# bbc/zipkin

Hardware: AMD Instinct MI355X
Metric: spans/sec into DependencyLinks (1/2/4/8 GPU) + % of HBM roofline (higher is better)
Workload: dtype u64

## Files before the change

### zipkin_amd/csrc/zk_api.cpp

```cpp
#include <hip/hip_runtime.h>
#include <string.h>

#include <new>
#include <string>
#include <utility>
#include <vector>

#include "zk_cluster.h"
#include "zk_comm.h"

#include "zk_internal.h"
#include "zk_launch.h"
#include "zk_lh_internal.h"
#include "zk_rl_internal.h"
#include "zk_rt_internal.h"

using namespace zk;

struct EventPair {
    hipEvent_t a = nullptr, b = nullptr;
};

struct zk_ctx {
    int device = 0;
// ... 47 lines not shown
    uint8_t* carry = nullptr;
    uint64_t carry_cap = 0;
    CarryState* cs = nullptr;
    bool maybe_carry = false;
    bool any_verify = false;
    std::string err;
    zk_rt* rt = nullptr;
    uint32_t rt_mode = ZK_RT_WITH_DEPS;
    zk_rl* rl = nullptr;
    zk_lh* lh = nullptr;
    std::vector<EventPair> ev_free, ev_join, ev_reduce, ev_spill, ev_fin, ev_cluster, ev_lh;
    zk_timing tm{};
};

namespace {

zk_status fail(zk_ctx* c, zk_status s, const std::string& msg) {
    if (c) c->err = msg;
    return s;
}

zk_status hip_fail(zk_ctx* c, hipError_t e, const char* where) {
    if (e == hipErrorLaunchOutOfResources && *launch_refusal())
        return fail(c, ZK_ERR_CAPACITY, std::string(where) + ": " + launch_refusal());
    return fail(c, ZK_ERR_HIP, std::string(where) + ": " + hipGetErrorString(e));
}

#define ZK_HIP(ctx, call)                                   \
    do {                                                    \
        hipError_t _e = (call);                             \
        if (_e != hipSuccess) return hip_fail(ctx, _e, #call); \
    } while (0)

#define ZK_ST(call)                        \
    do {                                   \
        const zk_status _s = (call);       \
        if (_s != ZK_OK) return _s;        \
    } while (0)

#define ZK_TRY try {
#define ZK_CATCH(ctx)                                                                      \
    }                                                                                      \
    catch (const std::bad_alloc&) {                                                        \
        return fail(ctx, ZK_ERR_CAPACITY, "host allocation failed");                       \
    }                                                                                      \
    catch (...) {                                                                          \
        return fail(ctx, ZK_ERR_INVALID_ARG, "unexpected host exception");                 \
    }

uint64_t table_bytes(uint32_t S) { return (uint64_t)S * S * kLimbs * 8 + kTableTailBytes; }

EventPair take_pair(zk_ctx* c) {
    EventPair p;
    if (!c->ev_free.empty()) {
        p = c->ev_free.back();
        c->ev_free.pop_back();
    } else {
        hipEventCreate(&p.a);
        hipEventCreate(&p.b);
    }
    return p;
}

uint64_t tiles_for(uint64_t n) { return (n + join_tile_records() - 1) / join_tile_records(); }

zk_status ensure_links(zk_ctx* c, uint32_t grid, uint64_t stride, uint64_t n) {
    const uint64_t slots = (uint64_t)grid * stride;
    const uint64_t sorted_slots = n + 64 < slots ? n + 64 : slots;
    const uint64_t sorted_bytes = sorted_slots * (reduce_compact(grid, stride) ? sizeof(uint32_t) : sizeof(uint64_t));
    const bool set_ok = slots <= c->link_slots && grid <= c->link_lists;
    const bool scratch_ok = !c->nb || (sorted_bytes <= c->sorted_bytes && grid <= c->col_off_lists);
    if (set_ok && scratch_ok) return ZK_OK;
    if (!set_ok) {
        hipFree(c->links);
        hipFree(c->link_count);
        hipFree(c->hist);
        c->links = nullptr;
        c->link_count = nullptr;
        c->hist = nullptr;
        c->link_slots = 0;
        c->link_lists = 0;
        ZK_HIP(c, hipMalloc(&c->links, slots * sizeof(uint64_t)));
        ZK_HIP(c, hipMalloc(&c->link_count, (uint64_t)grid * sizeof(uint32_t)));
        if (c->nb) ZK_HIP(c, hipMalloc(&c->hist, (uint64_t)grid * c->nb * sizeof(uint32_t)));
        c->link_slots = slots;
        c->link_lists = grid;
    }
    if (!scratch_ok) {
        const uint64_t sb = sorted_bytes > c->sorted_bytes ? sorted_bytes : c->sorted_bytes;
        const uint32_t gl = grid > c->col_off_lists ? grid : c->col_off_lists;
        hipFree(c->col_off);
        hipFree(c->sorted);
        c->col_off = nullptr;
        c->sorted = nullptr;
        c->sorted_bytes = 0;
        c->col_off_lists = 0;
        ZK_HIP(c, hipMalloc(&c->col_off, (uint64_t)gl * c->nb * sizeof(uint32_t)));
        ZK_HIP(c, hipMalloc(&c->sorted, sb));
        c->sorted_bytes = sb;
        c->col_off_lists = gl;
        if (!c->bucket_base) ZK_HIP(c, hipMalloc(&c->bucket_base, (c->nb + 1) * sizeof(uint64_t)));
    }
    return ZK_OK;
}

bool aligned(const void* p, uintptr_t a) { return ((uintptr_t)p & (a - 1)) == 0; }

zk_status ensure_spill(zk_ctx* c, uint64_t n) {
    const uint64_t need = tiles_for(n) + 1;
    if (need > c->spill_cap) {
        if (c->spill_list) ZK_HIP(c, hipFree(c->spill_list));
        uint64_t cap = need < (1ull << 16) ? (1ull << 16) : need;
        ZK_HIP(c, hipMalloc(&c->spill_list, cap * sizeof(uint64_t)));
        c->spill_cap = cap;
    }
    if (!c->spill_scratch) {
        c->spill_stride = spill_scratch_bytes_per_wg(c->max_trace);
        ZK_HIP(c, hipMalloc(&c->spill_scratch, c->spill_stride * c->spill_wgs));
    }
    return ZK_OK;
}

constexpr int kAbortShift = 48;
constexpr uint64_t kAbortUnit = 1ull << kAbortShift;

zk_status stats_sum(zk_ctx* c, uint64_t out[ST_N], uint64_t* aborted_ranks = nullptr) {
    const size_t bytes = (size_t)kStatShards * ST_N * 8;
    if (!c->h_stats) ZK_HIP(c, hipHostMalloc((void**)&c->h_stats, bytes, hipHostMallocDefault));
    if (!c->ev_stats) ZK_HIP(c, hipEventCreateWithFlags(&c->ev_stats, hipEventDisableTiming));
    const uint64_t cells = (uint64_t)c->S * c->S;
    if (c->merged)
        ZK_HIP(c, hipMemcpyAsync(c->h_stats, c->table + cells * kLimbs, kTableTailBytes, hipMemcpyDeviceToHost,
                                 c->stream));
    else
        ZK_HIP(c, hipMemcpyAsync(c->h_stats, c->stats, bytes, hipMemcpyDeviceToHost, c->stream));
    ZK_HIP(c, hipEventRecord(c->ev_stats, c->stream));
    hipError_t q;
    while ((q = hipEventQuery(c->ev_stats)) == hipErrorNotReady) {
    }
    if (q != hipSuccess) return fail(c, ZK_ERR_HIP, std::string("stats copy: ") + hipGetErrorString(q));
    const unsigned long long* h = c->h_stats;
    for (int s = 0; s < ST_N; ++s) out[s] = 0;
    for (int sh = 0; sh < (c->merged ? 1 : kStatShards); ++sh)
        for (int s = 0; s < ST_N; ++s) out[s] += h[(size_t)sh * ST_N + s];
    if (aborted_ranks) *aborted_ranks = out[ST_RECORDS] >> kAbortShift;
    out[ST_RECORDS] &= kAbortUnit - 1;
    return ZK_OK;
}

bool cols_ok(const zk_span_cols* c) {
    return c && c->trace_id && c->span_id && c->parent_id && c->first_ts && c->last_ts && c->service_id && c->flags;
}

uint64_t carved_bytes(uint64_t n) { return 5 * ((n * 8 + 255) & ~255ull) + 2 * ((n * 4 + 255) & ~255ull); }
SpanColsMut carve_cols(uint8_t* p, uint64_t n) {
    auto take = [&](uint64_t bytes) {
        uint8_t* q = p;
        p += (bytes + 255) & ~255ull;
        return q;
    };
    SpanColsMut m;
    m.trace_id = (uint64_t*)take(n * 8);
    m.span_id = (uint64_t*)take(n * 8);
    m.parent_id = (uint64_t*)take(n * 8);
    m.first_ts = (int64_t*)take(n * 8);
    m.last_ts = (int64_t*)take(n * 8);
    m.service_id = (uint32_t*)take(n * 4);
    m.flags = (uint32_t*)take(n * 4);
    return m;
}

zk_status ensure_cluster(zk_ctx* c, uint64_t n, const ClusterPlan& plan) {
    const uint64_t tb = cluster_scratch_bytes(plan);
    if (n > c->cl_cap) {
        hipFree(c->cl_cols);
        c->cl_cols = nullptr;
        c->cl_cap = 0;
        if (hipMalloc(&c->cl_cols, 2 * carved_bytes(n)) != hipSuccess) {
            (void)hipGetLastError();
            return fail(c, ZK_ERR_CAPACITY, "no device memory for the clustering pass (96 B per record)");
// ... 914 lines not shown
```

### zipkin_amd/csrc/zk_internal.h

```cpp
#pragma once
#include <hip/hip_runtime.h>
#include <stdint.h>

#include <string>

#include "../../include/zkagg.h"

#include <rocprofiler-sdk-roctx/roctx.h>
namespace zk {
struct RoctxRange {
    explicit RoctxRange(const char* name) { roctxRangePushA(name); }
    ~RoctxRange() { roctxRangePop(); }
    RoctxRange(const RoctxRange&) = delete;
    RoctxRange& operator=(const RoctxRange&) = delete;
};
}

namespace zk {

constexpr int kLimbs = 16;
constexpr int kLimbM0 = 0;
constexpr int kLimbS1 = 1;
constexpr int kLimbS2 = 3;
constexpr int kLimbS3 = 6;
// ... 24 lines not shown
    ST_RT_DUR_RANGE,
    ST_SPILL_OVERFLOW,
    ST_NOT_CLUSTERED,
    ST_N = 16
};
constexpr int kStatShards = 256;
constexpr uint64_t kTableTailBytes = ST_N * 8;
constexpr uint64_t kStatTailWords = ST_N;
static_assert(ST_NOT_CLUSTERED < ST_N, "stat slots");

struct SpanColsDev {
    const uint64_t* trace_id;
    const uint64_t* span_id;
    const uint64_t* parent_id;
    const int64_t* first_ts;
    const int64_t* last_ts;
    const uint32_t* service_id;
    const uint32_t* flags;
    uint64_t n;
};

struct JoinArgs {
    SpanColsDev c;
    uint64_t* table;
    unsigned long long* stats;
    uint32_t S;
    unsigned int* spill_count;
    uint64_t* spill_list;
    uint64_t spill_cap;
    uint8_t* spill_scratch;
    uint64_t spill_scratch_stride;
    uint32_t max_trace;
    uint64_t* links;
    uint32_t* link_count;
    uint64_t link_stride;
    uint64_t per_wg;
    uint32_t grid;
    uint32_t* hist;
    uint32_t nb;
    uint32_t cb_shift;
    uint32_t join;
    uint32_t skip;
    uint64_t* rt_pay;
    uint32_t* rt_svc;
    uint32_t* rt_count;
    unsigned long long* rt_dropped;
    uint64_t rt_spill_cap;
    uint64_t rt_seed;
    uint32_t rt_p;
    const uint32_t* sub;
    uint32_t nsub;
    uint32_t* big_list;
    unsigned int* big_count;
    const unsigned long long* n_dev;
    uint32_t append;
    const uint32_t* skip_dev;
    uint64_t* lk_key;
    uint64_t* lk_tid;
    uint32_t* lk_spill_count;
    uint64_t lk_spill_cap;
    uint32_t* lk_name;
    uint32_t* lh_hist;
    uint32_t lh_bins;
    uint32_t lh_m;
};

hipError_t launch_join(const JoinArgs& a, hipStream_t s, uint32_t blocks = 0);
hipError_t launch_group_join(const JoinArgs& a, hipStream_t s);
void group_join_geometry(uint64_t n, uint32_t cus, uint32_t* grid, uint64_t* per_wg, uint64_t* link_stride);
uint32_t group_join_capacity();
uint64_t join_tile_records();
void join_geometry(uint64_t n, uint32_t cus, uint32_t* grid, uint64_t* per_wg, uint64_t* link_stride);
hipError_t launch_link_reduce(const uint64_t* links, const uint32_t* counts, uint64_t stride, uint64_t tiles,
                              uint64_t* table, hipStream_t s);
#ifndef ZK_COMPACT_SLOT_LIMIT
#define ZK_COMPACT_SLOT_LIMIT 0x7FFFFFFFull
#endif
constexpr uint64_t kCompactSlotLimit = ZK_COMPACT_SLOT_LIMIT;
static_assert(kCompactSlotLimit <= 0x7FFFFFFFull, "an escape holds the slot in 31 bits, all ones is the pad");
constexpr uint32_t kCompactDurBits = 21;
constexpr uint32_t kCompactDurMask = (1u << kCompactDurBits) - 1;
constexpr uint32_t kCompactEscape = 0x80000000u;
constexpr uint32_t kCompactPad = 0xFFFFFFFFu;
bool reduce_compact(uint32_t lists, uint64_t stride);
struct ReduceArgs {
    const uint64_t* links;
    const uint32_t* counts;
    uint64_t stride;
    uint32_t lists;
    const uint32_t* hist;
    uint32_t nb, cb_shift;
    uint32_t* col_off;
    uint64_t* bucket_base;
    void* sorted;
    uint64_t* table;
    uint64_t cells;
    uint32_t compact;
};
hipError_t launch_partitioned_reduce(const ReduceArgs& r, hipStream_t s);
void bucket_geometry(uint32_t S, uint32_t* nb, uint32_t* cb_shift);
uint64_t reduce_scatter_dyn_lds(uint32_t S);
uint32_t scatter_lists_per_wg(uint32_t lists);
hipError_t launch_spill(const JoinArgs& a, uint32_t spill_wgs, hipStream_t s);
uint64_t spill_scratch_bytes_per_wg(uint32_t max_trace);
hipError_t launch_finalize(const uint64_t* table, uint32_t S, const zk_link_table* out,
                           hipStream_t s);
uint64_t exchange_bytes(uint32_t S);
hipError_t launch_table_pack(const uint64_t* table, uint32_t S, uint64_t* xchg, hipStream_t s);
hipError_t launch_table_unpack(const uint64_t* xchg, uint32_t S, uint64_t* table, hipStream_t s);
hipError_t launch_tracegen(const zk_tracegen_params* p, const zk_span_cols* out, uint64_t cap,
                           uint64_t* n_records, uint64_t* n_traces, hipStream_t s);

}
```

### zipkin_amd/csrc/zk_join.hip

```cpp
#include "zk_internal.h"
#include "zk_launch.h"
#include "zk_sketch_internal.h"

#ifndef ZK_HASH_FACTOR
#define ZK_HASH_FACTOR 8
#endif
#ifndef ZK_K1_WGS_PER_CU
#define ZK_K1_WGS_PER_CU 4
#endif
namespace zk {
namespace {

constexpr int kSpillWG = 256;

#ifdef ZK_STAMPS
__device__ unsigned long long g_zk_stamps[16];
__device__ __forceinline__ unsigned long long zk_memtime() {
    unsigned long long t;
    __builtin_amdgcn_sched_barrier(0);
    asm volatile("s_memtime %0\n\ts_waitcnt lgkmcnt(0)" : "=s"(t)::"memory");
    __builtin_amdgcn_sched_barrier(0);
    return t;
}
#define ZK_STAMP_DECL                                 \
// ... 215 lines not shown
__device__ __forceinline__ uint32_t lanes_below(uint64_t m) {
    return __builtin_amdgcn_mbcnt_hi((uint32_t)(m >> 32), __builtin_amdgcn_mbcnt_lo((uint32_t)m, 0u));
}

struct Window {
    uint64_t tid[2], sid[2], pid[2], first[2], last[2];
    uint32_t svc[2], flags[2];
    uint64_t prev;
};

__device__ __forceinline__ void window_ballots(const Window& w, uint64_t ws, int wn, uint64_t* ev, uint64_t* od) {
    const int t = threadIdx.x, lane = t & 63;
    uint64_t prev = lane_shr1(w.tid[1]);
    if (lane == 0) prev = (ws + 2 * t > 0) ? w.prev : ~w.tid[0];
    const bool b0 = (2 * t < wn) && w.tid[0] != prev;
    const bool b1 = (2 * t + 1 < wn) && w.tid[1] != w.tid[0];
    *ev = __ballot(b0);
    *od = __ballot(b1);
}

__device__ __forceinline__ void load_tid(const JoinArgs& a, uint64_t n, uint64_t ws, Window& w) {
    const uint64_t i = ws + 2 * threadIdx.x;
    ld2_u64(a.c.trace_id, i, n, w.tid);
    w.prev = a.c.trace_id[ZK_HOTIDX((i > 0 && i - 1 < n) ? i - 1 : 0)];
}
__device__ __forceinline__ void load_early(const JoinArgs& a, uint64_t n, uint64_t ws, Window& w) {
    const uint64_t i = ws + 2 * threadIdx.x;
    ld2_u64(a.c.span_id, i, n, w.sid);
#ifndef ZK_K1_DIAG_NOFIRST
    ld2_u64((const uint64_t*)a.c.first_ts, i, n, w.first);
#endif
    ld2_u64((const uint64_t*)a.c.last_ts, i, n, w.last);
#ifdef ZK_K1_DIAG_NOFIRST
    w.first[0] = w.last[0] - 5;
    w.first[1] = w.last[1] - 5;
#endif
    ld2_u32(a.c.service_id, i, n, w.svc);
}
template <bool JOIN>
__device__ __forceinline__ void load_late(const JoinArgs& a, uint64_t n, uint64_t ws, Window& w) {
    const uint64_t i = ws + 2 * threadIdx.x;
    if constexpr (JOIN) {
        ld2_u64(a.c.parent_id, i, n, w.pid);
    } else {
        w.pid[0] = w.pid[1] = 0ull;
    }
    ld2_u32(a.c.flags, i, n, w.flags);
}

constexpr int kModeJoin = 1;
constexpr int kModeEmit = 2;
constexpr int kModeLinks = 4;
template <int TILE, int WG, int MODE>
__global__ __launch_bounds__(WG, ZK_K1_WGS_PER_CU * WG / 256) void k_span_join_stream(JoinArgs a) {
    constexpr int H = ZK_HASH_FACTOR * TILE;
    constexpr int NWORD = TILE / 64;
    static_assert(TILE == 2 * WG && TILE <= 512, "two records per thread; the segment field of the slot word is 9 bits");
    __shared__ __align__(16) uint64_t s_sid[TILE];
    __shared__ __align__(16) long long s_first[TILE];
    __shared__ __align__(16) long long s_last[TILE];
    __shared__ __align__(16) uint64_t s_pid[TILE];
    __shared__ __align__(16) uint32_t s_svck[TILE];
    __shared__ __align__(16) uint32_t s_name[(MODE & kModeLinks) ? TILE / 2 : 1];
    __shared__ __align__(16) uint32_t s_ht[H];
    __shared__ __align__(16) uint64_t s_mask[NWORD];
    __shared__ uint32_t s_stat[ST_N];
    __shared__ uint64_t s_cursor;
    __shared__ uint32_t s_hist[kMaxBuckets];

    const int tid = threadIdx.x, lane = tid & 63, wave = tid >> 6;
    const uint64_t n = a.n_dev ? (uint64_t)*a.n_dev : a.c.n;
    uint64_t per = a.per_wg;
    if (a.n_dev) {
        const uint64_t q = ((n + a.grid - 1) / a.grid + TILE - 1) / TILE * TILE;
        if (q < per) per = q ? q : TILE;
    }
    const uint64_t R0 = (uint64_t)blockIdx.x * per;
    if (R0 >= n) {
        if (a.append) return;
        if (tid == 0) {
            a.link_count[blockIdx.x] = 0u;
            if (a.rt_count) a.rt_count[blockIdx.x] = 0u;
        }
        for (uint32_t x = tid; x < a.nb; x += WG) a.hist[(uint64_t)x * a.grid + blockIdx.x] = 0u;
        return;
    }
    const uint64_t R1 = (R0 + per < n) ? R0 + per : n;
    uint64_t* __restrict__ out = a.links + (uint64_t)blockIdx.x * a.link_stride;
    const uint64_t trash = a.link_stride - 1;
    uint64_t* __restrict__ it_pay = a.rt_pay + (uint64_t)blockIdx.x * a.link_stride;
    uint32_t* __restrict__ it_svc = a.rt_svc + (uint64_t)blockIdx.x * a.link_stride;
    uint64_t nrec = 0;
    StatPack st;
    int fold_in = kFoldWindows;
    if (tid < ST_N) s_stat[tid] = 0u;
    if (tid == 0) s_cursor = a.append ? (uint64_t)a.link_count[blockIdx.x] : 0ull;
    for (uint32_t x = tid; x < a.nb; x += WG) s_hist[x] = a.append ? a.hist[(uint64_t)x * a.grid + blockIdx.x] : 0u;
    constexpr uint32_t kNoSlot = 0xFFFFFFFFu;
    uint32_t r_clear[2] = {kNoSlot, kNoSlot};

    Window cur, nxt;
    constexpr bool JOIN = (MODE & kModeJoin) != 0, EMIT = (MODE & kModeEmit) != 0, LINKS = (MODE & kModeLinks) != 0;
    static_assert(!LINKS || (JOIN && !EMIT), "link items ride on the join's links");
#pragma unroll
    for (int x = tid; x < H / 4; x += WG) reinterpret_cast<uint4*>(s_ht)[x] = make_uint4(0u, 0u, 0u, 0u);
    uint64_t m_ev, m_od;
    ZK_STAMP_DECL
    uint64_t ws = R0;
    const uint32_t skip0 = a.skip_dev ? *a.skip_dev : a.skip;
    uint64_t seek = R0 + (blockIdx.x == 0 ? skip0 : 0u);
    bool seek_start = false;
    load_tid(a, n, ws, cur);
    load_early(a, n, ws, cur);
    window_ballots(cur, ws, (int)((n - ws) < (uint64_t)TILE ? (n - ws) : (uint64_t)TILE), &m_ev, &m_od);
    if (lane == 0) *reinterpret_cast<ulonglong2*>(&s_mask[2 * wave]) = make_ulonglong2(m_ev, m_od);
    for (;;) {
        load_late<JOIN>(a, n, ws, cur);
        const int wn = (int)((n - ws) < (uint64_t)TILE ? (n - ws) : (uint64_t)TILE);
        ZK_PHASE_SYNC(0);
        const int lo_j = (int)(seek - ws);
        const int r1_j = (R1 - ws < (uint64_t)wn) ? (int)(R1 - ws) : wn;
        int start = -1, stop = -1, last_b = -1, prev_b = -1;
        {
            constexpr int NW = WG / 64;
            uint64_t ev = 0ull, od = 0ull;
            if (lane < NW) {
                const ulonglong2 x = *reinterpret_cast<const ulonglong2*>(&s_mask[2 * lane]);
                ev = x.x;
                od = x.y;
            }
            const int base = 128 * lane;
            const bool fast = seek_start && lo_j < wn && R1 - ws >= (uint64_t)wn;
            if (fast) {
                start = lo_j;
            } else {
                const int fs = lane < NW ? first_ge(ev, od, lo_j - base) : -1;
                const int ft = lane < NW ? first_ge(ev, od, r1_j - base) : -1;
                const uint64_t bs = __ballot(fs >= 0), bt = __ballot(ft >= 0);
                if (bs) {
                    const int w = __ffsll((unsigned long long)bs) - 1;
                    start = 128 * w + __builtin_amdgcn_readlane(fs, w);
                }
                if (bt) {
                    const int w = __ffsll((unsigned long long)bt) - 1;
                    stop = 128 * w + __builtin_amdgcn_readlane(ft, w);
                }
            }
            const int lb = last_of(ev, od);
            const uint64_t bl = __ballot(lb >= 0);
            if (bl) {
                const int w = 63 - (int)__clzll((long long)bl);
                last_b = 128 * w + __builtin_amdgcn_readlane(lb, w);
            }
            const uint64_t bp = bl & ((1ull << wave) - 1ull);
            if (bp) {
                const int w = 63 - (int)__clzll((long long)bp);
                prev_b = 128 * w + __builtin_amdgcn_readlane(lb, w);
            }
        }
        const bool at_end = ws + (uint64_t)wn >= n;
        int m;
        bool done = false;
        uint64_t next_seek = 0;
        bool next_seek_start = false;
        if (start < 0 || (stop >= 0 && stop <= start)) {
            done = (start >= 0) || at_end || ws + (uint64_t)TILE >= R1;
            next_seek = ws + (uint64_t)TILE;
            start = m = 0;
        } else if (stop >= 0) {
            m = stop;
            done = true;
        } else if (at_end) {
            m = wn;
            done = true;
        } else if (last_b > start) {
            m = last_b;
            next_seek = ws + (uint64_t)last_b;
            next_seek_start = true;
        } else if (start > 1) {
            m = start;
// ... 214 lines not shown
        {
            const uint64_t wtot = (uint64_t)(__popcll(l1) + __popcll(l2)) | ((uint64_t)(__popcll(i1) + __popcll(i2)) << 32);
            uint64_t old = 0;
            if (lane == 0 && wtot) old = atomicAdd((unsigned long long*)&s_cursor, (unsigned long long)wtot);
            old = ((uint64_t)(uint32_t)__shfl((int)(uint32_t)(old >> 32), 0) << 32) | (uint32_t)__shfl((int)(uint32_t)old, 0);
            lbase = (uint32_t)old + lanes_below(l1) + lanes_below(l2);
            ibase = (uint32_t)(old >> 32) + lanes_below(i1) + lanes_below(i2);
        }
        if (!done) {
            const uint64_t nws = next_ws;
            window_ballots(nxt, nws, (int)((n - nws) < (uint64_t)TILE ? (n - nws) : (uint64_t)TILE), &n_ev, &n_od);
            if (lane == 0) *reinterpret_cast<ulonglong2*>(&s_mask[2 * wave]) = make_ulonglong2(n_ev, n_od);
        }
        if constexpr (JOIN) {
            uint32_t pos = lbase;
#if defined(ZK_K1_DIAG_TRASHONLY)
            out[trash] = r_link[0];
            out[trash] = r_link[1];
#elif !defined(ZK_K1_DIAG_NOSTORE)
#pragma unroll
            for (int e = 0; e < 2; ++e) {
                const bool v = (lm >> e) & 1u;
                const uint64_t at = v ? (uint64_t)pos : trash;
                out[at] = r_link[e];
                if constexpr (LINKS) {
                    a.lk_key[(uint64_t)blockIdx.x * a.link_stride + at] = r_lkey[e];
                    a.lk_tid[(uint64_t)blockIdx.x * a.link_stride + at] = cur.tid[e];
                    a.lk_name[(uint64_t)blockIdx.x * a.link_stride + at] = r_lname[e];
                }
                pos += v ? 1u : 0u;
            }
#else
            if (pos == 0xFFFFFFFFu) out[0] = r_link[0];
#endif
        }
        if constexpr (EMIT) {
            uint32_t pos = ibase;
#pragma unroll
            for (int e = 0; e < 2; ++e) {
                const bool v = r_item[e] != ~0ull;
                const uint64_t at = v ? (uint64_t)pos : trash;
                it_pay[at] = r_item[e];
                it_svc[at] = r_isvc[e];
                pos += v ? 1u : 0u;
            }
        }
#pragma unroll
        for (int e = 0; e < 2; ++e) r_clear[e] = (r_leader[e] == 2 * tid + e) ? r_slot[e] : kNoSlot;
        ZK_STAMP(6);
        if (--fold_in == 0) {
            fold_stats(st, s_stat);
            fold_in = kFoldWindows;
        }
        if (done) break;
        ws = next_ws;
        seek = next_seek;
        seek_start = next_seek_start;
        m_ev = n_ev;
        m_od = n_od;
        cur.tid[0] = nxt.tid[0];
        cur.tid[1] = nxt.tid[1];
        cur.prev = nxt.prev;
        ZK_STAMP(7);
    }
    ZK_STAMP_FLUSH();
    __syncthreads();
#ifdef ZK_K1_DIAG
    if (tid == 0) s_cursor = 0ull;
    for (uint32_t x = tid; x < a.nb; x += WG) s_hist[x] = 0u;
    __syncthreads();
#endif
    const uint32_t nout = (uint32_t)s_cursor;
    const uint32_t nitem = (uint32_t)(s_cursor >> 32);
    if (tid == 0) {
        a.link_count[blockIdx.x] = nout;
        if constexpr (EMIT) a.rt_count[blockIdx.x] = nitem;
        atomicAdd(&a.stats[(uint64_t)(blockIdx.x % kStatShards) * ST_N + ST_RECORDS], (unsigned long long)nrec);
    }
    fold_stats(st, s_stat);
    publish_stats(s_stat, a.stats);
    if constexpr (EMIT) {
        if (tid == 0 && s_stat[ST_RT_DUR_RANGE]) atomicAdd(&a.rt_dropped[1], (unsigned long long)s_stat[ST_RT_DUR_RANGE]);
    }
    if constexpr (JOIN) {
        for (uint32_t x = tid; x < a.nb; x += WG) a.hist[(uint64_t)x * a.grid + blockIdx.x] = s_hist[x];
    } else {
        for (uint32_t x = tid; x < a.nb; x += WG) a.hist[(uint64_t)x * a.grid + blockIdx.x] = 0u;
    }
}

struct SpillScratch {
    uint64_t* sid;
    long long* first;
    long long* last;
    uint64_t* cntA;
    uint64_t* cntB;
    uint64_t* pid;
    uint32_t* svck;
    uint32_t* name;
    uint32_t* ht;
};

__host__ __device__ inline uint64_t pow2ceil(uint64_t x) {
    uint64_t p = 1;
    while (p < x) p <<= 1;
    return p;
}

__host__ __device__ inline uint64_t spill_ht_slots(uint32_t max_trace) { return pow2ceil(2ull * max_trace); }

__host__ __device__ inline SpillScratch spill_carve(uint8_t* base, uint32_t L) {
    SpillScratch s;
    uint8_t* p = base;
    s.sid = (uint64_t*)p;
    p += 8ull * L;
    s.first = (long long*)p;
    p += 8ull * L;
    s.last = (long long*)p;
    p += 8ull * L;
    s.cntA = (uint64_t*)p;
    p += 8ull * L;
    s.cntB = (uint64_t*)p;
    p += 8ull * L;
    s.pid = (uint64_t*)p;
    p += 8ull * L;
    s.svck = (uint32_t*)p;
    p += 4ull * L + 4ull * (L & 1);
    s.name = (uint32_t*)p;
    p += 4ull * L + 4ull * (L & 1);
    s.ht = (uint32_t*)p;
    return s;
}

template <class T>
__device__ __forceinline__ T ld_sc(const T* p) {
    return __hip_atomic_load(p, __ATOMIC_RELAXED, __HIP_MEMORY_SCOPE_AGENT);
}
template <class T>
__device__ __forceinline__ void st_sc(T* p, T v) {
    __hip_atomic_store(p, v, __ATOMIC_RELAXED, __HIP_MEMORY_SCOPE_AGENT);
}

__device__ __forceinline__ void spill_counts(uint32_t f, uint64_t* A, uint64_t* B) {
    *A = (uint64_t)((f >> ZK_F_CS_SHIFT) & 3u) | ((uint64_t)((f >> ZK_F_CR_SHIFT) & 3u) << 21) |
         ((uint64_t)((f >> ZK_F_SR_SHIFT) & 3u) << 42);
    *B = (uint64_t)((f >> ZK_F_SS_SHIFT) & 3u) | ((uint64_t)(f & ZK_F_HAS_PARENT) << 21);
}
__device__ __forceinline__ bool spill_valid(uint64_t A, uint64_t B) {
    constexpr uint64_t F = (1ull << 21) - 1;
    return (A & F) <= 1 && ((A >> 21) & F) <= 1 && ((A >> 42) & F) <= 1 && (B & F) <= 1;
}

__global__ __launch_bounds__(kSpillWG) void k_span_join_spill(JoinArgs a) {
    __shared__ unsigned long long s_end;
    __shared__ unsigned long long s_stat[ST_N];
    const uint32_t total = min(*a.spill_count, (unsigned int)a.spill_cap);
    const uint64_t n = a.n_dev ? (uint64_t)*a.n_dev : a.c.n;
    const uint64_t* __restrict__ tr = a.c.trace_id;
    uint8_t* base = a.spill_scratch + (uint64_t)blockIdx.x * a.spill_scratch_stride;
    StatWide st;
    if (threadIdx.x < ST_N) s_stat[threadIdx.x] = 0u;
    for (uint32_t e = blockIdx.x; e < total; e += gridDim.x) {
        const uint64_t s = a.spill_list[e];
        const uint64_t t0 = tr[s];
        if (threadIdx.x == 0) s_end = ~0ull;
        __syncthreads();
        for (uint64_t b0 = s + 1;; b0 += kSpillWG) {
            const uint64_t i = b0 + threadIdx.x;
            if (i >= n || tr[i] != t0) atomicMin(&s_end, (unsigned long long)i);
            __syncthreads();
            const uint64_t e_now = s_end;
// ... 433 lines not shown
                    const uint64_t osid = s_sid[oi];
                    const uint64_t otid = s_tid[oi];
                    const uint32_t osvc = s_svck[oi];
                    if (osid == pL && otid == cur.tid[e]) {
                        pw = o;
                        sp = osvc;
                        break;
                    }
                }
                slot = (slot + 1) & (kGH - 1);
            }
            if (pw == 0u || !slot_valid(pw)) {
                st.inc(ST_MISSING_PARENT);
                continue;
            }
            st.inc(ST_JOINED);
            if (sp == kSvcNone || sL == kSvcNone) {
                st.inc(ST_NO_SERVICE);
                continue;
            }
            const uint64_t d = (uint64_t)(s_last[j] - s_first[j]);
            if (d >= kMaxDuration) {
                st.inc(ST_DUR_RANGE);
                continue;
            }
            const uint64_t cell = (uint64_t)(sp & kSvcIdMask) * a.S + (sL & kSvcIdMask);
            r_link[e] = (cell << 40) | d;
            if (a.nb) atomicAdd(&s_hist[cell >> a.cb_shift], 1u);
            lm |= 1u << e;
        }
        ZK_STAMP(4);
        ld2_u64(a.c.trace_id, nbase + 2 * threadIdx.x, a.c.n, cur.tid);
        ld2_u64(a.c.parent_id, nbase + 2 * threadIdx.x, a.c.n, cur.pid);
        ld2_u32(a.c.flags, nbase + 2 * threadIdx.x, a.c.n, cur.flags);
        const uint64_t l1 = __ballot(lm != 0u), l2 = __ballot(lm == 3u);
        uint32_t lbase = 0;
        {
            const uint32_t wtot = (uint32_t)(__popcll(l1) + __popcll(l2));
            uint32_t old = 0;
            if (lane == 0 && wtot) old = atomicAdd(&s_cursor, wtot);
            lbase = (uint32_t)__shfl((int)old, 0) + lanes_below(l1) + lanes_below(l2);
        }
        uint32_t pos = lbase;
#pragma unroll
        for (int e = 0; e < 2; ++e) {
            const bool v = (lm >> e) & 1u;
            out[v ? (uint64_t)pos : trash] = r_link[e];
            pos += v ? 1u : 0u;
        }
#pragma unroll
        for (int e = 0; e < 2; ++e) r_clear[e] = (r_leader[e] == j0 + e) ? r_slot[e] : kNoSlot;
        if (--fold_in == 0) {
            fold_stats(st, s_stat);
            fold_in = kFoldWindows;
        }
        ZK_PHASE_SYNC(5);
    };

    Window wa, wb;
    uint32_t la = 0, ha = 0, lb = 0, hb = 0;
    gs = next_batch(gs, bv, &la, &ha);
    if (ha > la) load_group(a, la & ~1u, wa);
    bv = fetch(gs);
    gs = next_batch(gs, bv, &lb, &hb);
    if (hb > lb) load_group(a, lb & ~1u, wb);
    bv = fetch(gs);
    ZK_STAMP(6);
    for (;;) {
        if (ha <= la) break;
        run_group(wa, la, ha, &la, &ha);
        ZK_STAMP(6);
        if (hb <= lb) break;
        run_group(wb, lb, hb, &lb, &hb);
        ZK_STAMP(6);
    }
    ZK_STAMP_FLUSH();
    __syncthreads();
    if (tid == 0) {
        a.link_count[blockIdx.x] = s_cursor;
        atomicAdd(&a.stats[(uint64_t)(blockIdx.x % kStatShards) * ST_N + ST_RECORDS], (unsigned long long)nrec);
    }
    fold_stats(st, s_stat);
    publish_stats(s_stat, a.stats);
    for (uint32_t x = tid; x < a.nb; x += kGWG) a.hist[(uint64_t)x * a.grid + blockIdx.x] = s_hist[x];
}

#ifndef ZK_K1_WG
#define ZK_K1_WG 256
#endif
constexpr int kTileWG = ZK_K1_WG;
constexpr int kTile = 2 * kTileWG;

}

uint64_t spill_scratch_bytes_per_wg(uint32_t max_trace) {
    const uint64_t L = max_trace;
    uint64_t b = 8ull * L * 6 + 2 * (4ull * L + 4ull * (L & 1)) + 4ull * spill_ht_slots(max_trace);
    return (b + 255) & ~255ull;
}

hipError_t launch_join(const JoinArgs& a, hipStream_t s, uint32_t blocks) {
    if (a.c.n == 0) return hipSuccess;
    const dim3 g((unsigned)(blocks ? blocks : a.grid)), b(kTileWG);
    const bool emit = a.rt_pay != nullptr, join = a.join != 0;
    if (a.lk_key && join && !emit)
        return launch_checked("k_span_join_stream<join|links>", k_span_join_stream<kTile, kTileWG, kModeJoin | kModeLinks>,
                              g, b, 0, s, a);
    if (emit && join)
        return launch_checked("k_span_join_stream<join|emit>", k_span_join_stream<kTile, kTileWG, kModeJoin | kModeEmit>,
                              g, b, 0, s, a);
    if (emit)
        return launch_checked("k_span_join_stream<emit>", k_span_join_stream<kTile, kTileWG, kModeEmit>, g, b, 0, s, a);
    return launch_checked("k_span_join_stream<join>", k_span_join_stream<kTile, kTileWG, kModeJoin>, g, b, 0, s, a);
}

hipError_t launch_spill(const JoinArgs& a, uint32_t spill_wgs, hipStream_t s) {
    if (a.c.n == 0) return hipSuccess;
    return launch_checked("k_span_join_spill", k_span_join_spill, dim3(spill_wgs), dim3(kSpillWG), 0, s, a);
}

uint64_t join_tile_records() { return kTile; }

hipError_t launch_group_join(const JoinArgs& a, hipStream_t s) {
    if (a.c.n == 0) return hipSuccess;
    return launch_checked("k_group_join", k_group_join, dim3(a.grid), dim3(kGWG), 0, s, a);
}

uint32_t group_join_capacity() { return kGCap; }

void group_join_geometry(uint64_t n, uint32_t cus, uint32_t* grid, uint64_t* per_wg, uint64_t* link_stride) {
    uint64_t g = (uint64_t)(cus ? cus : 256) * kGPerCU;
    const uint64_t by_n = (n + kGCap - 1) / kGCap;
    if (g > by_n) g = by_n ? by_n : 1;
    const uint64_t per = (n + g - 1) / g;
    *grid = (uint32_t)g;
    *per_wg = per ? per : 1;
    const uint64_t fb = (*per_wg + kTile - 1) / kTile * kTile + kTile;
    *link_stride = *per_wg + kGCap + fb + 1;
}

#ifdef ZK_STAMPS
extern "C" int zk_debug_stamps(unsigned long long* out, int reset) {
    if (hipMemcpyFromSymbol(out, HIP_SYMBOL(g_zk_stamps), 16 * 8) != hipSuccess) return 1;
    if (reset) {
        unsigned long long z[16] = {0};
        if (hipMemcpyToSymbol(HIP_SYMBOL(g_zk_stamps), z, sizeof(z)) != hipSuccess) return 1;
    }
    return 0;
}
#endif

void join_geometry(uint64_t n, uint32_t cus, uint32_t* grid, uint64_t* per_wg, uint64_t* link_stride) {
    const uint64_t windows = (n + kTile - 1) / kTile;
#ifndef ZK_K1_GRID_MULT
#define ZK_K1_GRID_MULT 4
#endif
    uint64_t g = (uint64_t)cus * ZK_K1_WGS_PER_CU * ZK_K1_GRID_MULT;
    if (g > windows) g = windows ? windows : 1;
    const uint64_t per = ((n + g - 1) / g + kTile - 1) / kTile * kTile;
    *grid = (uint32_t)g;
    *per_wg = per ? per : kTile;
    *link_stride = *per_wg + kTile + 1;
}}
```

### zipkin_amd/csrc/zk_reduce.hip

```cpp
#include <type_traits>

#include "zk_block.h"
#include "zk_internal.h"
#include "zk_launch.h"

#ifndef ZK_K2U
#define ZK_K2U 8
#endif
constexpr int kK2U = ZK_K2U;
constexpr int kK2WG = 1024;
constexpr int kK3U = 4;

namespace zk {
namespace {

__device__ __forceinline__ uint64_t limb_value(int q, uint64_t d) {
    constexpr uint64_t M = 0xFFFFFFFFull;
    if (q == kLimbM0) return 1;
    if (q < kLimbS2) return (d >> (32 * (q - kLimbS1))) & M;
    const unsigned __int128 d2 = (unsigned __int128)d * d;
    if (q < kLimbS3) return (uint64_t)(d2 >> (32 * (q - kLimbS2))) & M;
    const unsigned __int128 d3 = d2 * d;
    if (q < kLimbS4) return (uint64_t)(d3 >> (32 * (q - kLimbS3))) & M;
    const uint64_t lo = (uint64_t)d3, hi = (uint64_t)(d3 >> 64);
    const unsigned __int128 p0 = (unsigned __int128)lo * d;
    const unsigned __int128 p1 = (unsigned __int128)hi * d + (uint64_t)(p0 >> 64);
    const int c = q - kLimbS4;
    if (c < 2) return ((uint64_t)p0 >> (32 * c)) & M;
    return (uint64_t)(p1 >> (32 * (c - 2))) & M;
}

__global__ __launch_bounds__(256) void k_link_reduce_atomic(const uint64_t* __restrict__ links,
                                                            const uint32_t* __restrict__ counts, uint64_t stride,
                                                            uint64_t tiles, uint64_t* __restrict__ table) {
    const int q = threadIdx.x & 15;
    const int g = threadIdx.x >> 4;
    for (uint64_t t = blockIdx.x; t < tiles; t += gridDim.x) {
        const uint32_t c = counts[t];
        const uint64_t* L = links + t * stride;
        for (uint32_t i = g; i < c; i += 16) {
            const uint64_t v = L[i];
            const uint64_t cell = v >> 40, d = v & (kMaxDuration - 1);
            if (q < 15) {
                const uint64_t x = limb_value(q, d);
                if (x) atomicAdd((unsigned long long*)(table + cell * kLimbs + q), (unsigned long long)x);
            }
        }
    }
}


__global__ __launch_bounds__(1024) void k_bucket_colscan(const uint32_t* __restrict__ hist, uint32_t lists,
                                                         uint32_t* __restrict__ col_off, uint64_t* __restrict__ totals) {
    __shared__ uint32_t s_tmp[32];
    const uint32_t b = blockIdx.x;
    uint64_t carry = 0;
    for (uint32_t base = 0; base < lists; base += 1024) {
        const uint32_t w = base + threadIdx.x;
        const uint32_t v = w < lists ? hist[(uint64_t)b * lists + w] : 0u;
        uint32_t tot;
        const uint32_t ex = block_excl_scan<16>(v, s_tmp, &tot);
        if (w < lists) col_off[(uint64_t)b * lists + w] = (uint32_t)carry + ex;
        carry += tot;
        __syncthreads();
    }
    if (threadIdx.x == 0) totals[b] = carry;
}

__global__ __launch_bounds__(1024) void k_bucket_base(uint64_t* __restrict__ base, uint32_t nb) {
    __shared__ uint32_t s_tmp[32];
    const uint32_t b = threadIdx.x;
    const uint32_t v = b < nb ? (uint32_t)base[b] : 0u;
    uint32_t tot;
    const uint32_t ex = block_excl_scan<16>(v, s_tmp, &tot);
    __syncthreads();
    if (b < nb) base[b] = ex;
    if (b == 0) base[nb] = tot;
}

constexpr int kScatterLineBytes = 64;
constexpr int kScatterMaxLPW = 16;
constexpr uint32_t kScatterGrid = 256;
template <int U, int WG, bool COMPACT>
__global__ __launch_bounds__(WG) void k_link_scatter(ReduceArgs r, uint32_t lpw) {
    constexpr int C = WG * U;
    using W = typename std::conditional<COMPACT, uint32_t, uint64_t>::type;
    constexpr uint32_t kScatterLine = kScatterLineBytes / sizeof(W);
    __shared__ uint32_t s_pre[kScatterMaxLPW + 4];
    __shared__ uint32_t s_cur[kMaxBuckets];
    __shared__ uint32_t s_hist[kMaxBuckets];
    __shared__ uint32_t s_off[kMaxBuckets];
    __shared__ uint32_t s_cc[kMaxBuckets];
    __shared__ uint2 s_ld[kMaxBuckets];
    __shared__ W s_sorted[C];
    __shared__ uint16_t s_tag[COMPACT ? C : 1];
    __shared__ uint32_t s_tmp[32];
    extern __shared__ __attribute__((aligned(16))) uint64_t s_carry_raw[];
    W* const s_carry = reinterpret_cast<W*>(s_carry_raw);
    W* const out = static_cast<W*>(r.sorted);
    const uint32_t gx = gridDim.x / 8, gr = gridDim.x % 8, xi = blockIdx.x % 8;
    const uint32_t w = (xi * gx + (xi < gr ? xi : gr) + blockIdx.x / 8) * lpw;
    const uint32_t nl = (r.lists - w) < lpw ? (r.lists - w) : lpw;
    const int tid = threadIdx.x;
    constexpr int BPT = (kMaxBuckets + WG - 1) / WG;
    for (uint32_t b = tid; b < r.nb; b += WG) {
        s_cur[b] = (uint32_t)r.bucket_base[b] + r.col_off[(uint64_t)b * r.lists + w];
        s_hist[b] = 0u;
        s_cc[b] = 0u;
    }
    if (tid == 0) {
        uint32_t acc = 0;
        for (uint32_t q = 0; q < nl; ++q) {
            s_pre[q] = acc;
            acc += r.counts[w + q];
        }
        s_pre[nl] = acc;
        for (uint32_t q = nl + 1; q < kScatterMaxLPW + 4; ++q) s_pre[q] = 0xFFFFFFFFu;
    }
    __syncthreads();
    const uint32_t c = s_pre[nl];
    uint32_t pre[kScatterMaxLPW + 1];
#pragma unroll
    for (int q = 0; q <= kScatterMaxLPW; ++q) pre[q] = q <= (int)nl ? s_pre[q] : 0xFFFFFFFFu;
    auto at = [&](uint32_t i) -> const uint64_t* {
        uint32_t q = 0;
#pragma unroll
        for (int k = 1; k < kScatterMaxLPW; ++k) q += (i >= pre[k]) ? 1u : 0u;
        q = q < nl - 1 ? q : nl - 1;
        return r.links + (uint64_t)(w + q) * r.stride + (i - pre[q]);
    };
    auto escape_of = [&](uint32_t i) -> uint32_t {
        uint32_t q = 0;
        while (q + 1 < nl && i >= s_pre[q + 1]) ++q;
        return kCompactEscape | (uint32_t)((uint64_t)(w + q) * r.stride + (i - s_pre[q]));
    };
    uint32_t q0 = 0;
    auto load_chunk = [&](uint64_t (&dst)[U], uint32_t b0) {
        if (b0 >= c) {
#pragma unroll
            for (int k = 0; k < U; ++k) dst[k] = r.links[(uint64_t)w * r.stride];
            return;
        }
        while (q0 + 1 < nl && b0 >= s_pre[q0 + 1]) ++q0;
        const uint32_t pa = s_pre[q0], p1 = s_pre[q0 + 1], p2 = s_pre[q0 + 2], p3 = s_pre[q0 + 3];
        if ((uint64_t)b0 + C <= p3) {
#pragma unroll
            for (int k = 0; k < U; ++k) {
                const uint32_t i = b0 + tid + WG * k;
                const uint32_t ii = i < c ? i : b0;
                const uint32_t q = q0 + (ii >= p1 ? 1u : 0u) + (ii >= p2 ? 1u : 0u);
                const uint32_t lo = ii >= p2 ? p2 : (ii >= p1 ? p1 : pa);
                dst[k] = r.links[(uint64_t)(w + q) * r.stride + (ii - lo)];
            }
        } else {
#pragma unroll
            for (int k = 0; k < U; ++k) {
                const uint32_t i = b0 + tid + WG * k;
                dst[k] = *at(i < c ? i : 0);
            }
        }
    };
    uint64_t nxt[U];
    load_chunk(nxt, 0u);
    for (uint32_t base = 0; base < c; base += C) {
        const uint32_t cnt = (c - base) < (uint32_t)C ? (c - base) : (uint32_t)C;
        const bool last = base + C >= c;
        uint64_t raw[U];
        W v[U];
        uint32_t bk[U], rank[U];
#pragma unroll
        for (int k = 0; k < U; ++k) raw[k] = nxt[k];
        load_chunk(nxt, base + C);
#pragma unroll
        for (int k = 0; k < U; ++k) {
            const uint32_t cell = (uint32_t)(raw[k] >> 40);
            bk[k] = cell >> r.cb_shift;
            const bool in = tid + WG * k < (int)cnt;
            if constexpr (COMPACT) {
                const uint64_t d = raw[k] & (kMaxDuration - 1);
                v[k] = ((cell - (bk[k] << r.cb_shift)) << kCompactDurBits) | (uint32_t)d;
                if (in && d > kCompactDurMask) v[k] = escape_of(base + tid + WG * k);
            } else {
                v[k] = raw[k];
            }
            rank[k] = in ? atomicAdd(&s_hist[bk[k]], 1u) : 0u;
        }
        __syncthreads();
        {
            uint32_t h[BPT], sum = 0;
// ... 362 lines not shown
            limb[1] = S1 & M;
            limb[2] = S1 >> 32;
            limb[3] = (uint64_t)S2 & M;
            limb[4] = ((uint64_t)S2) >> 32;
            limb[5] = (uint64_t)(S2 >> 64);
            limb[6] = (uint64_t)s3lo & M;
            limb[7] = ((uint64_t)s3lo) >> 32;
            limb[8] = (uint64_t)(s3lo >> 64) & M;
            limb[9] = ((uint64_t)(s3lo >> 96)) | (s3hi << 32);
            limb[10] = s4w0 & M;
            limb[11] = s4w0 >> 32;
            limb[12] = s4w1 & M;
            limb[13] = s4w1 >> 32;
            limb[14] = s4w2;
        }
        __syncthreads();
#pragma unroll
        for (int q = 0; q < 15; ++q) s_t[tid * CS + q] = limb[q];
        __syncthreads();
        for (int x = tid; x < CB * kLimbs; x += WG) {
            const int c = x >> 4, q = x & 15;
            const uint64_t cell = cell0 + c;
            if (cell >= r.cells || q == 15) continue;
            const uint64_t v = s_t[c * CS + q];
            if (!v) continue;
            uint64_t* dst = r.table + cell * kLimbs + q;
            if (splits == 1)
                *dst += v;
            else
                atomicAdd((unsigned long long*)dst, (unsigned long long)v);
        }
        __syncthreads();
        if (s1 >= p1) break;
    }
}

}

constexpr uint32_t kCbMinShift = 9;

void bucket_geometry(uint32_t S, uint32_t* nb, uint32_t* cb_shift) {
    const uint64_t cells = (uint64_t)S * S;
    *nb = 0;
    *cb_shift = 0;
    for (uint32_t sh = kCbMinShift; sh <= 10; ++sh) {
        const uint64_t n = (cells + (1ull << sh) - 1) >> sh;
        if (n <= kMaxBuckets) {
            *nb = (uint32_t)n;
            *cb_shift = sh;
            return;
        }
    }
}

uint64_t reduce_scatter_dyn_lds(uint32_t S) {
    uint32_t nb = 0, sh = 0;
    bucket_geometry(S, &nb, &sh);
    return (uint64_t)nb * kScatterLineBytes;
}

uint32_t scatter_lists_per_wg(uint32_t lists) {
    const uint32_t lpw = (lists + kScatterGrid - 1) / kScatterGrid;
    return lpw > (uint32_t)kScatterMaxLPW ? (uint32_t)kScatterMaxLPW : lpw;
}

bool reduce_compact(uint32_t lists, uint64_t stride) { return (uint64_t)lists * stride < kCompactSlotLimit; }

namespace {
template <bool COMPACT>
hipError_t launch_scatter_reduce(const ReduceArgs& r, uint32_t k2_grid, uint32_t lpw, uint32_t splits, hipStream_t s) {
    const hipError_t e = launch_checked("k_link_scatter", k_link_scatter<kK2U, kK2WG, COMPACT>, dim3(k2_grid), dim3(kK2WG),
                                        (size_t)r.nb * kScatterLineBytes, s, r, lpw);
    if (e != hipSuccess) return e;
    if (r.cb_shift == 9)
        return launch_checked("k_bucket_lds_reduce_wide<9>", k_bucket_lds_reduce_wide<9, 512, COMPACT>,
                              dim3(r.nb * splits), dim3(512), 0, s, r, splits);
    return launch_checked("k_bucket_reduce<10>", k_bucket_reduce<10, 4, COMPACT>, dim3(r.nb * splits), dim3(1024), 0, s, r,
                          splits);
}
}

hipError_t launch_partitioned_reduce(const ReduceArgs& r, hipStream_t s) {
    if (!r.nb || !r.lists) return hipSuccess;
    hipError_t e = launch_checked("k_bucket_colscan", k_bucket_colscan, dim3(r.nb), dim3(1024), 0, s, r.hist, r.lists,
                                  r.col_off, r.bucket_base);
    if (e != hipSuccess) return e;
    e = launch_checked("k_bucket_base", k_bucket_base, dim3(1), dim3(1024), 0, s, r.bucket_base, r.nb);
    if (e != hipSuccess) return e;
    const uint32_t lpw = scatter_lists_per_wg(r.lists);
    const uint32_t k2_grid = (r.lists + lpw - 1) / lpw;
    const uint32_t splits = r.nb >= 256 ? 1u : (512u + r.nb - 1) / r.nb;
    return r.compact ? launch_scatter_reduce<true>(r, k2_grid, lpw, splits, s)
                     : launch_scatter_reduce<false>(r, k2_grid, lpw, splits, s);
}

hipError_t launch_link_reduce(const uint64_t* links, const uint32_t* counts, uint64_t stride, uint64_t tiles,
                              uint64_t* table, hipStream_t s) {
    if (!tiles) return hipSuccess;
    const uint64_t grid = tiles < 4096 ? tiles : 4096;
    return launch_checked("k_link_reduce_atomic", k_link_reduce_atomic, dim3((unsigned)grid), dim3(256), 0, s, links,
                          counts, stride, tiles, table);
}

}
```

Measured before the change: 75.74 billion.

## Transpose bucket histogram to row-per-list layout and use segmented two-pass column scan

The per-workgroup bucket histogram and column offsets move from bucket-major to list-major layout, with rows padded to a multiple of 32 words. Join kernels now write contiguous rows, and the scatter kernel reads its offsets contiguously. The single-block-per-bucket column scan becomes a two-pass segmented scan (column sums, then scan with carries) using vectorized uint4 loads across 16 segments, which raises parallelism when the number of lists is large. The cost is an extra kernel launch and a slightly larger col_off allocation to hold the segment totals.

```diff
diff --git a/zipkin_amd/csrc/zk_api.cpp b/zipkin_amd/csrc/zk_api.cpp
--- a/zipkin_amd/csrc/zk_api.cpp
+++ b/zipkin_amd/csrc/zk_api.cpp
@@ -153,7 +153,7 @@
         c->link_lists = 0;
         ZK_HIP(c, hipMalloc(&c->links, slots * sizeof(uint64_t)));
         ZK_HIP(c, hipMalloc(&c->link_count, (uint64_t)grid * sizeof(uint32_t)));
-        if (c->nb) ZK_HIP(c, hipMalloc(&c->hist, (uint64_t)grid * c->nb * sizeof(uint32_t)));
+        if (c->nb) ZK_HIP(c, hipMalloc(&c->hist, (uint64_t)grid * hist_row_words(c->nb) * sizeof(uint32_t)));
         c->link_slots = slots;
         c->link_lists = grid;
     }
@@ -166,7 +166,7 @@
         c->sorted = nullptr;
         c->sorted_bytes = 0;
         c->col_off_lists = 0;
-        ZK_HIP(c, hipMalloc(&c->col_off, (uint64_t)gl * c->nb * sizeof(uint32_t)));
+        ZK_HIP(c, hipMalloc(&c->col_off, ((uint64_t)gl + kScanSegs) * hist_row_words(c->nb) * sizeof(uint32_t)));
         ZK_HIP(c, hipMalloc(&c->sorted, sb));
         c->sorted_bytes = sb;
         c->col_off_lists = gl;
diff --git a/zipkin_amd/csrc/zk_internal.h b/zipkin_amd/csrc/zk_internal.h
--- a/zipkin_amd/csrc/zk_internal.h
+++ b/zipkin_amd/csrc/zk_internal.h
@@ -130,6 +130,8 @@
 constexpr uint32_t kCompactDurMask = (1u << kCompactDurBits) - 1;
 constexpr uint32_t kCompactEscape = 0x80000000u;
 constexpr uint32_t kCompactPad = 0xFFFFFFFFu;
+__host__ __device__ inline uint32_t hist_row_words(uint32_t nb) { return (nb + 31u) & ~31u; }
+constexpr uint32_t kScanSegs = 16;
 bool reduce_compact(uint32_t lists, uint64_t stride);
 struct ReduceArgs {
     const uint64_t* links;
diff --git a/zipkin_amd/csrc/zk_join.hip b/zipkin_amd/csrc/zk_join.hip
--- a/zipkin_amd/csrc/zk_join.hip
+++ b/zipkin_amd/csrc/zk_join.hip
@@ -321,7 +321,7 @@
             a.link_count[blockIdx.x] = 0u;
             if (a.rt_count) a.rt_count[blockIdx.x] = 0u;
         }
-        for (uint32_t x = tid; x < a.nb; x += WG) a.hist[(uint64_t)x * a.grid + blockIdx.x] = 0u;
+        for (uint32_t x = tid; x < hist_row_words(a.nb); x += WG) a.hist[(uint64_t)blockIdx.x * hist_row_words(a.nb) + x] = 0u;
         return;
     }
     const uint64_t R1 = (R0 + per < n) ? R0 + per : n;
@@ -334,7 +334,7 @@
     int fold_in = kFoldWindows;
     if (tid < ST_N) s_stat[tid] = 0u;
     if (tid == 0) s_cursor = a.append ? (uint64_t)a.link_count[blockIdx.x] : 0ull;
-    for (uint32_t x = tid; x < a.nb; x += WG) s_hist[x] = a.append ? a.hist[(uint64_t)x * a.grid + blockIdx.x] : 0u;
+    for (uint32_t x = tid; x < a.nb; x += WG) s_hist[x] = a.append ? a.hist[(uint64_t)blockIdx.x * hist_row_words(a.nb) + x] : 0u;
     constexpr uint32_t kNoSlot = 0xFFFFFFFFu;
     uint32_t r_clear[2] = {kNoSlot, kNoSlot};
 
@@ -715,11 +715,8 @@
     if constexpr (EMIT) {
         if (tid == 0 && s_stat[ST_RT_DUR_RANGE]) atomicAdd(&a.rt_dropped[1], (unsigned long long)s_stat[ST_RT_DUR_RANGE]);
     }
-    if constexpr (JOIN) {
-        for (uint32_t x = tid; x < a.nb; x += WG) a.hist[(uint64_t)x * a.grid + blockIdx.x] = s_hist[x];
-    } else {
-        for (uint32_t x = tid; x < a.nb; x += WG) a.hist[(uint64_t)x * a.grid + blockIdx.x] = 0u;
-    }
+    uint32_t* const row = a.hist + (uint64_t)blockIdx.x * hist_row_words(a.nb);
+    for (uint32_t x = tid; x < hist_row_words(a.nb); x += WG) row[x] = (JOIN && x < a.nb) ? s_hist[x] : 0u;
 }
 
 struct SpillScratch {
@@ -1319,7 +1316,8 @@
     }
     fold_stats(st, s_stat);
     publish_stats(s_stat, a.stats);
-    for (uint32_t x = tid; x < a.nb; x += kGWG) a.hist[(uint64_t)x * a.grid + blockIdx.x] = s_hist[x];
+    uint32_t* const row = a.hist + (uint64_t)blockIdx.x * hist_row_words(a.nb);
+    for (uint32_t x = tid; x < hist_row_words(a.nb); x += kGWG) row[x] = x < a.nb ? s_hist[x] : 0u;
 }
 
 #ifndef ZK_K1_WG
diff --git a/zipkin_amd/csrc/zk_reduce.hip b/zipkin_amd/csrc/zk_reduce.hip
--- a/zipkin_amd/csrc/zk_reduce.hip
+++ b/zipkin_amd/csrc/zk_reduce.hip
@@ -49,22 +49,116 @@
     }
 }
 
-
-__global__ __launch_bounds__(1024) void k_bucket_colscan(const uint32_t* __restrict__ hist, uint32_t lists,
-                                                         uint32_t* __restrict__ col_off, uint64_t* __restrict__ totals) {
-    __shared__ uint32_t s_tmp[32];
-    const uint32_t b = blockIdx.x;
-    uint64_t carry = 0;
-    for (uint32_t base = 0; base < lists; base += 1024) {
-        const uint32_t w = base + threadIdx.x;
-        const uint32_t v = w < lists ? hist[(uint64_t)b * lists + w] : 0u;
-        uint32_t tot;
-        const uint32_t ex = block_excl_scan<16>(v, s_tmp, &tot);
-        if (w < lists) col_off[(uint64_t)b * lists + w] = (uint32_t)carry + ex;
-        carry += tot;
-        __syncthreads();
-    }
-    if (threadIdx.x == 0) totals[b] = carry;
+constexpr int kScanWG = 256;
+constexpr int kScanK = 4;
+constexpr int kScanChunk = (kScanWG / 8) * kScanK;
+
+__device__ __forceinline__ uint4 add4(uint4 a, uint4 b) { return make_uint4(a.x + b.x, a.y + b.y, a.z + b.z, a.w + b.w); }
+__device__ __forceinline__ uint4 sub4(uint4 a, uint4 b) { return make_uint4(a.x - b.x, a.y - b.y, a.z - b.z, a.w - b.w); }
+
+__device__ __forceinline__ void scan_load(const uint32_t* __restrict__ hist, uint32_t row_words, uint32_t col, uint32_t w0,
+                                          uint32_t end, uint4 (&v)[kScanK]) {
+#pragma unroll
+    for (int k = 0; k < kScanK; ++k) {
+        const uint32_t w = w0 + k;
+        v[k] = w < end ? *reinterpret_cast<const uint4*>(hist + (uint64_t)w * row_words + col) : make_uint4(0u, 0u, 0u, 0u);
+    }
+}
+__device__ __forceinline__ void scan_segment(uint32_t lists, uint32_t seg, uint32_t* lo, uint32_t* hi) {
+    const uint32_t per = (lists + kScanSegs - 1) / kScanSegs;
+    *lo = seg * per < lists ? seg * per : lists;
+    *hi = *lo + per < lists ? *lo + per : lists;
+}
+
+__global__ __launch_bounds__(kScanWG) void k_bucket_colsum(const uint32_t* __restrict__ hist, uint32_t lists, uint32_t nb,
+                                                           uint32_t* __restrict__ seg_tot) {
+    constexpr int NW = kScanWG / 64;
+    __shared__ uint4 s_w[NW][8];
+    const uint32_t row_words = hist_row_words(nb);
+    const int tid = threadIdx.x, lane = tid & 63, wave = tid >> 6;
+    const uint32_t c4 = tid & 7, r0 = tid >> 3;
+    const uint32_t col = blockIdx.x * 32 + c4 * 4;
+    uint32_t lo, hi;
+    scan_segment(lists, blockIdx.y, &lo, &hi);
+    uint4 sum = make_uint4(0u, 0u, 0u, 0u), nxt[kScanK];
+    scan_load(hist, row_words, col, lo + r0 * kScanK, hi, nxt);
+    for (uint32_t base = lo; base < hi; base += kScanChunk) {
+        uint4 cur[kScanK];
+#pragma unroll
+        for (int k = 0; k < kScanK; ++k) cur[k] = nxt[k];
+        if (base + kScanChunk < hi) scan_load(hist, row_words, col, base + kScanChunk + r0 * kScanK, hi, nxt);
+#pragma unroll
+        for (int k = 0; k < kScanK; ++k) sum = add4(sum, cur[k]);
+    }
+#pragma unroll
+    for (int d = 8; d < 64; d <<= 1)
+        sum = add4(sum, make_uint4(__shfl_xor(sum.x, d), __shfl_xor(sum.y, d), __shfl_xor(sum.z, d), __shfl_xor(sum.w, d)));
+    if (lane < 8) s_w[wave][c4] = sum;
+    __syncthreads();
+    if (tid < 8) {
+        uint4 t = s_w[0][tid];
+#pragma unroll
+        for (int v = 1; v < NW; ++v) t = add4(t, s_w[v][tid]);
+        *reinterpret_cast<uint4*>(seg_tot + (uint64_t)blockIdx.y * row_words + col) = t;
+    }
+}
+
+__global__ __launch_bounds__(kScanWG) void k_bucket_colscan(const uint32_t* __restrict__ hist, uint32_t lists, uint32_t nb,
+                                                            const uint32_t* __restrict__ seg_tot, uint32_t* __restrict__ col_off,
+                                                            uint64_t* __restrict__ totals) {
+    constexpr int NW = kScanWG / 64;
+    __shared__ uint4 s_w[2][NW][8];
+    const uint32_t row_words = hist_row_words(nb);
+    const int tid = threadIdx.x, lane = tid & 63, wave = tid >> 6;
+    const uint32_t c4 = tid & 7, r0 = tid >> 3;
+    const uint32_t col = blockIdx.x * 32 + c4 * 4;
+    const uint32_t seg = blockIdx.y;
+    const uint4 zero = make_uint4(0u, 0u, 0u, 0u);
+    uint32_t lo, hi;
+    scan_segment(lists, seg, &lo, &hi);
+    uint4 nxt[kScanK];
+    scan_load(hist, row_words, col, lo + r0 * kScanK, hi, nxt);
+    uint4 carry = zero;
+    for (uint32_t q = 0; q < seg; ++q) carry = add4(carry, *reinterpret_cast<const uint4*>(seg_tot + (uint64_t)q * row_words + col));
+    int par = 0;
+    for (uint32_t base = lo; base < hi; base += kScanChunk, par ^= 1) {
+        uint4 cur[kScanK], ex[kScanK], run = zero;
+#pragma unroll
+        for (int k = 0; k < kScanK; ++k) cur[k] = nxt[k];
+        if (base + kScanChunk < hi) scan_load(hist, row_words, col, base + kScanChunk + r0 * kScanK, hi, nxt);
+#pragma unroll
+        for (int k = 0; k < kScanK; ++k) {
+            ex[k] = run;
+            run = add4(run, cur[k]);
+        }
+        uint4 inc = run;
+#pragma unroll
+        for (int d = 8; d < 64; d <<= 1) {
+            const uint4 t = make_uint4(__shfl_up(inc.x, d), __shfl_up(inc.y, d), __shfl_up(inc.z, d), __shfl_up(inc.w, d));
+            if (lane >= d) inc = add4(inc, t);
+        }
+        if (lane >= 56) s_w[par][wave][c4] = inc;
+        __syncthreads();
+        uint4 pre = add4(carry, sub4(inc, run)), tot = zero;
+#pragma unroll
+        for (int v = 0; v < NW; ++v) {
+            const uint4 x = s_w[par][v][c4];
+            if (v < wave) pre = add4(pre, x);
+            tot = add4(tot, x);
+        }
+        carry = add4(carry, tot);
+#pragma unroll
+        for (int k = 0; k < kScanK; ++k) {
+            const uint32_t w = base + r0 * kScanK + k;
+            if (w < hi) *reinterpret_cast<uint4*>(col_off + (uint64_t)w * row_words + col) = add4(pre, ex[k]);
+        }
+    }
+    if (seg == kScanSegs - 1 && r0 == 0) {
+        const uint32_t t[4] = {carry.x, carry.y, carry.z, carry.w};
+#pragma unroll
+        for (int i = 0; i < 4; ++i)
+            if (col + i < nb) totals[col + i] = t[i];
+    }
 }
 
 __global__ __launch_bounds__(1024) void k_bucket_base(uint64_t* __restrict__ base, uint32_t nb) {
@@ -104,7 +198,7 @@
     const int tid = threadIdx.x;
     constexpr int BPT = (kMaxBuckets + WG - 1) / WG;
     for (uint32_t b = tid; b < r.nb; b += WG) {
-        s_cur[b] = (uint32_t)r.bucket_base[b] + r.col_off[(uint64_t)b * r.lists + w];
+        s_cur[b] = (uint32_t)r.bucket_base[b] + r.col_off[(uint64_t)w * hist_row_words(r.nb) + b];
         s_hist[b] = 0u;
         s_cc[b] = 0u;
     }
@@ -633,8 +727,12 @@
 
 hipError_t launch_partitioned_reduce(const ReduceArgs& r, hipStream_t s) {
     if (!r.nb || !r.lists) return hipSuccess;
-    hipError_t e = launch_checked("k_bucket_colscan", k_bucket_colscan, dim3(r.nb), dim3(1024), 0, s, r.hist, r.lists,
-                                  r.col_off, r.bucket_base);
+    const dim3 sg(hist_row_words(r.nb) / 32, kScanSegs);
+    uint32_t* const seg_tot = r.col_off + (uint64_t)r.lists * hist_row_words(r.nb);
+    hipError_t e = launch_checked("k_bucket_colsum", k_bucket_colsum, sg, dim3(kScanWG), 0, s, r.hist, r.lists, r.nb, seg_tot);
+    if (e != hipSuccess) return e;
+    e = launch_checked("k_bucket_colscan", k_bucket_colscan, sg, dim3(kScanWG), 0, s, r.hist, r.lists, r.nb,
+                       (const uint32_t*)seg_tot, r.col_off, r.bucket_base);
     if (e != hipSuccess) return e;
     e = launch_checked("k_bucket_base", k_bucket_base, dim3(1), dim3(1024), 0, s, r.bucket_base, r.nb);
     if (e != hipSuccess) return e;
```

Result: no change. 76.17 billion, median of 2 (+0.6%).
